# KVM-Explorer/AscendPathTracing

Hardware: AMD Instinct MI355X
Metric: Mray/s (ray segments per second) at 1920x1080, 8 bounces, 256 spp, demo scene (higher is better)
Workload: dtype f32; 1 GPU; C2: gen_spheres() 8-sphere scene, 1920x1080, S=64 (256 spp), depth 8, rays generated on device (counter RNG, seed 0), K-mode arithmetic, all segments traced (no retirement); segments_per_gpu=4246732800, parallelism=single GPU

## Files before the change

ascendpathtracing_amd/csrc/apt_host.h:

```cpp
#pragma once
#include <stdint.h>

#include <mutex>

#include "../../include/render_mi355x.h"

#define APT_API __attribute__((visibility("default")))

namespace apt {

void clear_error();
int set_error(int code, const char *fmt, const char *detail = "");

constexpr uint32_t kDefaultRefillLanes = 32;
constexpr int kMaxStatusDevices = 16;

struct Debug {
    uint32_t queue_ppw = 0;
    uint32_t queue_nbuf = 0;
    uint32_t queue_lds_pad = 0;
    uint32_t grid_walk = 0;
    double grid_spheres_per_cell = 0;
};

}

struct apt_context {
    struct Values {
        apt_render_params params;
        unsigned long long *trace_counter;
        uint32_t refill_lanes;
        apt::Debug debug;
        bool has_camera = false;
        apt_camera camera;
    };
    apt_context();
    Values snapshot();
    void set_params(const apt_render_params &p);
    void set_trace_counter(unsigned long long *c);
    void set_refill_lanes(uint32_t lanes);
    void set_camera(const apt_camera *cam_or_null);
    int set_debug(const char *key, double value);
    int get_debug(const char *key, double *value);
// ... 15 lines not shown
```

ascendpathtracing_amd/csrc/host_helpers.cpp:

```cpp
#include <stdint.h>
#include <stdio.h>
#include <string.h>

#include <algorithm>
#include <cmath>
#include <cstdlib>
#include <vector>

#include <string>

#include "../../include/render_mi355x.h"
#include "apt_host.h"
#include "pt_core.h"
#include "pt_camera.h"
#include "pt_leaf.h"

namespace {
thread_local std::string t_err;
thread_local int t_status = APT_OK;
}

namespace apt {
void clear_error() { t_err.clear(); t_status = APT_OK; }
int set_error(int code, const char *fmt, const char *detail) {
// ... 3 lines not shown
    t_status = code;
    return code;
}
apt_context &default_context() {
    static apt_context ctx;
    return ctx;
}
}

namespace {
double env_number(const char *name) {
    const char *e = getenv(name);
    return e ? atof(e) : 0.0;
}
}

apt_context::apt_context() {
    apt_default_params(&v_.params);
    v_.trace_counter = nullptr;
    v_.refill_lanes = apt::kDefaultRefillLanes;
    v_.has_camera = false;
    memset(&v_.camera, 0, sizeof v_.camera);
    struct { const char *env, *key; } knobs[] = {{"APT_QUEUE_PPW", "queue_ppw"}, {"APT_QUEUE_NBUF", "queue_nbuf"}, {"APT_QUEUE_LDS_PAD", "queue_lds_pad"},
                                                 {"APT_GRID_SPHERES_PER_CELL", "grid_spheres_per_cell"}};
    for (const auto &k : knobs) {
        const double v = env_number(k.env);
        if (v != 0.0) (void)set_debug(k.key, v);
    }
    if (const char *e = getenv("APT_GRID_WALK")) if (e[0] == 'i') v_.debug.grid_walk = 1;
    apt::clear_error();
}
apt_context::Values apt_context::snapshot() { std::lock_guard<std::mutex> g(m_); return v_; }
void apt_context::set_params(const apt_render_params &p) { std::lock_guard<std::mutex> g(m_); v_.params = p; }
void apt_context::set_trace_counter(unsigned long long *c) { std::lock_guard<std::mutex> g(m_); v_.trace_counter = c; }
void apt_context::set_refill_lanes(uint32_t lanes) { std::lock_guard<std::mutex> g(m_); v_.refill_lanes = lanes; }
void apt_context::set_camera(const apt_camera *cam) {
    std::lock_guard<std::mutex> g(m_);
    v_.has_camera = cam != nullptr;
    if (cam) v_.camera = *cam;
}
int apt_context::set_debug(const char *key, double value) {
    if (!key) return apt::set_error(APT_ERR_ARG, "apt_context_set_debug: key is null%s");
    const std::string k(key);
    const bool whole = value == std::floor(value);
    std::lock_guard<std::mutex> g(m_);
    apt::Debug &d = v_.debug;
    if (k == "queue_ppw") { if (!(whole && value >= 0 && value <= 4096)) goto range; d.queue_ppw = (uint32_t)value; }
    else if (k == "queue_nbuf") { if (!(whole && (value == 0 || (value >= 2 && value <= 16)))) goto range; d.queue_nbuf = (uint32_t)value; }
    else if (k == "queue_lds_pad") { if (!(whole && value >= 0 && value <= 32768)) goto range; d.queue_lds_pad = (uint32_t)value; }
    else if (k == "grid_walk") { if (!(value == 0 || value == 1)) goto range; d.grid_walk = (uint32_t)value; }
    else if (k == "grid_spheres_per_cell") { if (!(value == 0 || (value > 0.01 && value < 1e6))) goto range; d.grid_spheres_per_cell = value; }
    else return apt::set_error(APT_ERR_ARG, "apt_context_set_debug: unknown key '%s'", key);
    return APT_OK;
range:
    return apt::set_error(APT_ERR_ARG, "apt_context_set_debug: value out of range for '%s'", key);
}
int apt_context::get_debug(const char *key, double *value) {
    if (!key) return apt::set_error(APT_ERR_ARG, "apt_context_get_debug: key is null%s");
    const std::string k(key);
    std::lock_guard<std::mutex> g(m_);
    const apt::Debug &d = v_.debug;
    if (k == "queue_ppw") *value = d.queue_ppw;
    else if (k == "queue_nbuf") *value = d.queue_nbuf;
    else if (k == "queue_lds_pad") *value = d.queue_lds_pad;
    else if (k == "grid_walk") *value = d.grid_walk;
    else if (k == "grid_spheres_per_cell") *value = d.grid_spheres_per_cell;
    else return apt::set_error(APT_ERR_ARG, "apt_context_get_debug: unknown key '%s'", key);
    return APT_OK;
}
uint32_t *apt_context::status_lookup(int dev) {
    if (dev < 0 || dev >= apt::kMaxStatusDevices) return nullptr;
    std::lock_guard<std::mutex> g(m_);
    return status_[dev];
}
uint32_t *apt_context::status_adopt(int dev, uint32_t *fresh, uint32_t **spare) {
    *spare = nullptr;
    if (dev < 0 || dev >= apt::kMaxStatusDevices) { *spare = fresh; return nullptr; }
    std::lock_guard<std::mutex> g(m_);
    if (status_[dev]) *spare = fresh;
    else status_[dev] = fresh;
    return status_[dev];
}
void apt_context::status_release(uint32_t *out[apt::kMaxStatusDevices]) {
    std::lock_guard<std::mutex> g(m_);
    for (int i = 0; i < apt::kMaxStatusDevices; ++i) { out[i] = status_[i]; status_[i] = nullptr; }
}

// ... 531 lines not shown
```

ascendpathtracing_amd/csrc/materials.hip:

```cpp
#include <hip/hip_runtime.h>
#include <stdint.h>
#include <string.h>

#include <algorithm>

#include "../../include/render_mi355x.h"
#include "apt_materials.h"
#include "pt_core.h"
#include "pt_dispatch.h"
#include "pt_materials.h"

namespace {

TraceArgs mat_trace_args(const apt::MatTrace &t) {
    TraceArgs ta;
    ta.ns = t.ns; ta.depth = t.depth; ta.light = t.light;
    ta.eps = t.eps; ta.gain = 0.0f; ta.traced = t.traced;
    ta.status = t.status;
    ta.refill_lanes = (uint32_t)(uintptr_t)t.lights;
    ta.grid = t.grid;
    ta.grid_walk = 0;
    ta.emission = (uint32_t)((uint64_t)(uintptr_t)t.lights >> 32);
    ta.rr_start = t.rr_start;
    ta.seed = t.seed;
// ... 35 lines not shown
    }
    if (acc) atomicAdd(res, acc);
    if (rej) atomicAdd(res + 1, rej);
    if (bad) atomicAdd(res + 2, bad);
    if (ray_rej) atomicAdd(res + 3, ray_rej);
    if (max_cert) atomicMax(res + 4, max_cert);
}

}

namespace apt {

void selftest_direction(void *stream, const double *d3, uint64_t count, uint64_t *result5, uint8_t *flags) {
    const uint64_t blocks = std::min<uint64_t>((count + kBlock - 1) / kBlock, 256 * 16);
    hipLaunchKernelGGL(selftest_direction_kernel, dim3((unsigned)blocks), dim3(kBlock), 0, (hipStream_t)stream, d3, count,
                       (unsigned long long *)result5, flags);
}

void mat_render_frame(const MatFrameCall &c) {
    FrameArgs fa;
    CameraEx cx;
    if (c.camera) { cx = camera_ex(*c.camera, c.width, c.height); fa.cam = cx.base; }
    else camera_init(fa.cam, c.width, c.height);
    fa.width = c.width; fa.height = c.height; fa.samples = c.samples; fa.seed = c.t.seed;
    fa.pixel_begin = c.pixel_begin; fa.pixel_count = c.pixel_count; fa.fb = c.fb; fa.fb_u8 = c.fb_u8;
    const TraceArgs ta = mat_trace_args(c.t);
    LeafProg lp;
    (void)make_leaf_plan(c.samples, lp);
    if (c.camera) memcpy(&lp.leaf[kCamTailLeaf], &cx.t, sizeof cx.t);
    const int group = c.samples >= 8 ? 8 : 1;
    const uint64_t blocks = (c.pixel_count * 4u * (uint64_t)group + kBlock - 1) / kBlock;
    const size_t lds = lp.nleaves > 1 ? (size_t)kMaxStack * 3 * kStackSlots * sizeof(float) : 0;
    hipStream_t st = (hipStream_t)c.stream;
    with_flag(c.t.ns == 8, [&](auto ns8) { with_flag(c.t.grid != nullptr, [&](auto gr) { with_flag(group == 8, [&](auto g8) {
        with_flag(c.t.nee, [&](auto nee) { with_flag(c.t.lights != nullptr, [&](auto lt) { with_flag(c.camera != nullptr, [&](auto cam) {
            hipLaunchKernelGGL((render_frame_mat_kernel<mat_scene_form(ns8, gr, nee, lt, cam), g8 ? 8 : 1>), dim3((unsigned)blocks), dim3(kBlock), lds,
                               st, c.spheres, c.materials, fa, ta, lp);
        }); }); });
    }); }); });
}

void mat_render_paths(const MatPathsCall &c) {
    const TraceArgs ta = mat_trace_args(c.t);
    const uint64_t blocks = (c.c + kBlock - 1) / kBlock;
    hipStream_t st = (hipStream_t)c.stream;
    with_flag(c.t.ns == 8, [&](auto ns8) { with_flag(c.t.grid != nullptr, [&](auto gr) {
        with_flag(c.t.nee, [&](auto nee) { with_flag(c.t.lights != nullptr, [&](auto lt) {
// ... 20 lines not shown
```

ascendpathtracing_amd/csrc/pt_core.h:

```cpp
#pragma once
#include <stdint.h>
#include <cmath>
#include <cstdlib>
#include <cstring>
#include <math.h>

#if defined(__HIPCC__)
#include <hip/hip_runtime.h>
#define APT_HD __host__ __device__ __forceinline__
#else
#define APT_HD inline
#endif

namespace apt {

constexpr int kModeKernel = 0;
constexpr int kModeOracle = 1;
constexpr float kMissT = 1e20f;

APT_HD float intersect_sphere(float cx, float cy, float cz, float r2, float ox, float oy, float oz, float dx, float dy,
                              float dz, float eps) {
    float ocx = cx - ox, ocy = cy - oy, ocz = cz - oz;
    float b = ocx * dx;
    b = b + ocy * dy;
// ... 371 lines not shown
    uint32_t b;
    memcpy(&b, &f, sizeof b);
    return b;
#endif
}
APT_HD uint32_t dir_probe(double d0, double d1, double d2, double y, float e0, float e1, float e2, double &cert) {
    double q0, q1, q2, Z;
    uint32_t mid;
    fast_direction(d0, d1, d2, norm3_sq(d0, d1, d2), y, q0, q1, q2, Z, cert, mid);
    const bool ray = (fabs(d0) >= 0x1p-60) & (fabs(d1) >= 0x1p-60) & (fabs(d2) >= 0x1p-60) & (Z >= 0x1p-60) & (fabs(cert) <= kDirCertTau);
    uint32_t r = ray ? 64u : 0u;
    r |= (ray & (dir_mid_key(q0) > 16u * kDirMidD)) ? 1u : 0u;
    r |= (ray & (dir_mid_key(q1) > 16u * kDirMidD)) ? 2u : 0u;
    r |= (ray & (dir_mid_key(q2) > 16u * kDirMidD)) ? 4u : 0u;
    r |= float_bits((float)q0) != float_bits(e0) ? 8u : 0u;
    r |= float_bits((float)q1) != float_bits(e1) ? 16u : 0u;
    r |= float_bits((float)q2) != float_bits(e2) ? 32u : 0u;
    return r;
}
struct RayCheck { double lo, cert; uint32_t mid; };
APT_HD bool ray_check_ok(const RayCheck &k) { return (k.lo >= 0x1p-60) & (fabs(k.cert) <= kDirCertTau) & (k.mid > 16u * kDirMidD); }
APT_HD bool ray_check_ok_rn(const RayCheck &k) { return (k.lo >= 0x1p-60) & (k.cert <= 0x1p60); }

template <bool FAST, bool RSQDIR = true, class CAM>
APT_HD void camera_ray_t(const CAM &c, uint32_t w, uint32_t h, uint32_t i, uint32_t j, uint32_t sy, uint32_t sx,
                         double u1, double u2, float &rox, float &roy, float &roz, float &rdx, float &rdy, float &rdz, RayCheck &chk) {
    double arg1, arg2;
    const double ddx = tent_t<FAST>(u1, arg1), ddy = tent_t<FAST>(u2, arg2);
    const double xa = ((double)sx + 0.5 + ddx) / 2 + (double)i, xb = ((double)sy + 0.5 + ddy) / 2 + (double)j;
    double a, b;
#if defined(__HIP_DEVICE_COMPILE__)
    if (FAST) {
        a = div_by_rn_reciprocal(xa, (double)w, c.inv_w) - 0.5;
        b = div_by_rn_reciprocal(xb, (double)h, c.inv_h) - 0.5;
    } else
#endif
    {
        a = xa / (double)w - 0.5;
        b = xb / (double)h - 0.5;
    }
    const double d0 = cam_cx0(c) * a;
    const double d1 = cam_cy1(c) * b + cam_g1(c);
    const double d2 = cam_cy2(c) * b + cam_g2(c);
    const double n2 = norm3_sq(d0, d1, d2);
    rox = (float)(c.pos[0] + d0 * 140);
    roy = (float)(c.pos[1] + d1 * 140);
    roz = (float)(c.pos[2] + d2 * 140);
#if defined(__HIP_DEVICE_COMPILE__)
// ... 8 lines not shown
        lo = min3_abs_f64(lo, d1, d2);
        asm("v_min_f64 %0, %1, %2" : "=v"(lo) : "v"(lo), "v"(n2));
        chk.lo = lo; chk.cert = n;
        return;
    }
    if (FAST) {
        double q0, q1, q2, Z;
        fast_direction(d0, d1, d2, n2, __builtin_amdgcn_rsq(n2), q0, q1, q2, Z, chk.cert, chk.mid);
        rdx = (float)q0; rdy = (float)q1; rdz = (float)q2;
        double lo = min3_abs_f64(arg1, arg2, xa);
        lo = min3_abs_f64(lo, xb, d0);
        lo = min3_abs_f64(lo, d1, d2);
        asm("v_min_f64 %0, %1, %2" : "=v"(lo) : "v"(lo), "v"(Z));
        chk.lo = lo;
        return;
    }
#endif
    const double n = sqrt(n2);
    rdx = (float)(d0 / n);
    rdy = (float)(d1 / n);
    rdz = (float)(d2 / n);
}

template <bool RSQDIR = true, class CAM>
APT_HD void camera_ray(const CAM &c, uint32_t w, uint32_t h, uint32_t i, uint32_t j, uint32_t sy, uint32_t sx,
                       double u1, double u2, float &rox, float &roy, float &roz, float &rdx, float &rdy, float &rdz) {
    RayCheck chk;
#if defined(__HIP_DEVICE_COMPILE__)
    camera_ray_t<true, RSQDIR>(c, w, h, i, j, sy, sx, u1, u2, rox, roy, roz, rdx, rdy, rdz, chk);
    if (__builtin_expect(__builtin_amdgcn_ballot_w64(!(RSQDIR ? ray_check_ok(chk) : ray_check_ok_rn(chk))) == 0, 1)) return;
    asm volatile("" ::: "memory");
#endif
    camera_ray_t<false>(c, w, h, i, j, sy, sx, u1, u2, rox, roy, roz, rdx, rdy, rdz, chk);
}
APT_HD Ray camera_ray(const Camera &c, uint32_t w, uint32_t h, uint32_t i, uint32_t j, uint32_t sy, uint32_t sx,
                      double u1, double u2) {
    Ray r;
    camera_ray(c, w, h, i, j, sy, sx, u1, u2, r.ox, r.oy, r.oz, r.dx, r.dy, r.dz);
    return r;
}

APT_HD uint64_t splitmix64(uint64_t x) {
    x += 0x9E3779B97F4A7C15ull;
    x = (x ^ (x >> 30)) * 0xBF58476D1CE4E5B9ull;
    x = (x ^ (x >> 27)) * 0x94D049BB133111EBull;
    return x ^ (x >> 31);
}
APT_HD uint64_t xorshift64s(uint64_t &s) {
// ... 12 lines not shown
    return d - 1.0;
#endif
}
constexpr uint64_t kPathStride = 0x3C6EF372FE94F82Aull;
APT_HD void path_uniforms_at(uint64_t state, double &u1, double &u2) {
    u1 = unit_from_bits(splitmix64(state));
    u2 = unit_from_bits(splitmix64(state + 0x9E3779B97F4A7C15ull));
}
APT_HD void path_uniforms(uint64_t seed, uint64_t path, double &u1, double &u2) {
    path_uniforms_at(splitmix64(seed) + path * kPathStride, u1, u2);
}

constexpr uint64_t kPairStateStep = 8ull * kPathStride;
APT_HD uint64_t lane_base_state(uint64_t seed, uint64_t pbase, uint32_t j) { return splitmix64(seed) + (pbase + j) * kPathStride; }
APT_HD uint64_t chain_state_uniform(uint64_t lane_base, uint32_t u) {
    uint64_t off = (uint64_t)u * kPathStride;
#if defined(__HIP_DEVICE_COMPILE__)
    asm("" : "+s"(off));
#endif
    return lane_base + off;
}

#if defined(__HIPCC__)
template <class CAM>
__device__ __forceinline__ void camera_ray_pair(const CAM &c, uint32_t w, uint32_t h, uint32_t i, uint32_t j, uint32_t sy, uint32_t sx,
                                                uint64_t state_a, f2 &ox, f2 &oy, f2 &oz, f2 &dx, f2 &dy, f2 &dz) {
#if defined(__HIP_DEVICE_COMPILE__)
    double u1a, u2a, u1b, u2b;
    path_uniforms_at(state_a, u1a, u2a);
    path_uniforms_at(state_a + kPairStateStep, u1b, u2b);
    float ax, ay, az, adx, ady, adz, bx, by, bz, bdx, bdy, bdz;
    RayCheck ka, kb;
    camera_ray_t<true>(c, w, h, i, j, sy, sx, u1a, u2a, ax, ay, az, adx, ady, adz, ka);
    camera_ray_t<true>(c, w, h, i, j, sy, sx, u1b, u2b, bx, by, bz, bdx, bdy, bdz, kb);
    double lo;
    asm("v_min_f64 %0, %1, %2" : "=v"(lo) : "v"(ka.lo), "v"(kb.lo));
    const bool ok = (lo >= 0x1p-60) & (fabs(ka.cert) <= kDirCertTau) & (fabs(kb.cert) <= kDirCertTau) &
                    ((ka.mid < kb.mid ? ka.mid : kb.mid) > 16u * kDirMidD);
    if (__builtin_expect(__builtin_amdgcn_ballot_w64(!ok) != 0, 0)) {
        asm volatile("" ::: "memory");
        camera_ray_t<false>(c, w, h, i, j, sy, sx, u1a, u2a, ax, ay, az, adx, ady, adz, ka);
        camera_ray_t<false>(c, w, h, i, j, sy, sx, u1b, u2b, bx, by, bz, bdx, bdy, bdz, kb);
    }
    ox = f2{ax, bx}; oy = f2{ay, by}; oz = f2{az, bz};
    dx = f2{adx, bdx}; dy = f2{ady, bdy}; dz = f2{adz, bdz};
#endif
}
#endif
// ... 172 lines not shown
```

ascendpathtracing_amd/csrc/pt_frame.h:

```cpp
#pragma once
#include "pt_trace.h"

namespace {

struct FrameArgs {
    Camera cam;
    uint32_t width, height, samples;
    uint64_t seed;
    uint64_t pixel_begin, pixel_count;
    float *fb;
    uint8_t *fb_u8;
};

__device__ __forceinline__ void park_camera(Camera &cam, const FrameArgs &fa) {
    if (threadIdx.x < sizeof(Camera) / sizeof(double)) (&cam.pos[0])[threadIdx.x] = (&fa.cam.pos[0])[threadIdx.x];
}

template <int GROUP>
struct FrameLane {
    uint32_t j, sub;
    uint64_t pl;
    bool valid;
    uint64_t q;
    uint32_t pi, pj, sy, sx;
    uint64_t pbase;
};
template <int GROUP>
__device__ __forceinline__ FrameLane<GROUP> frame_lane(const FrameArgs &fa, uint32_t tid = threadIdx.x) {
    FrameLane<GROUP> f;
    const uint64_t L = (uint64_t)xcd_chunked_block<16>(blockIdx.x, gridDim.x) * kBlock + tid;
    f.j = (GROUP == 8) ? (uint32_t)(L & 7) : 0u;
    f.sub = (uint32_t)(L / GROUP) & 3u;
    f.pl = L / (4 * GROUP);
    f.valid = f.pl < fa.pixel_count;
    f.q = fa.pixel_begin + (f.valid ? f.pl : 0);
    f.pi = (uint32_t)(f.q / fa.height); f.pj = (uint32_t)(f.q % fa.height);
    f.sy = f.sub >> 1; f.sx = f.sub & 1;
    f.pbase = (f.q * 4 + f.sub) * fa.samples;
    return f;
}

constexpr uint32_t frame_u8_words(int group) { return kBlock / (4 * group) * 3 / 4; }
template <int GROUP>
__device__ __forceinline__ void frame_decode(const FrameArgs fa, uint64_t pl, bool valid, const float (&res)[3],
                                             uint32_t (&u8pack_kernel)[frame_u8_words(GROUP)]) {
    constexpr uint32_t kPixPerBlock = kBlock / (4 * GROUP), kU8Words = frame_u8_words(GROUP);
    typedef __attribute__((address_space(3))) uint8_t lds_uint8;
    typedef __attribute__((address_space(3))) uint32_t lds_uint32;
    lds_uint32 *const u8pack = (lds_uint32 *)u8pack_kernel;
    static_assert(kPixPerBlock * 3 % 4 == 0, "a workgroup's 8-bit pixels are whole dwords");
    const uint32_t lane = threadIdx.x & 63;
    const uint64_t pl0 = pl - (threadIdx.x / (4 * GROUP));
    const bool pack = fa.fb_u8 && pl0 + kPixPerBlock <= fa.pixel_count && (((uintptr_t)fa.fb_u8 + pl0 * 3) & 3u) == 0;
    const float fs = (float)fa.samples;
    const int gbase = (int)(lane & ~(uint32_t)(4 * GROUP - 1));
#pragma unroll
    for (int ch = 0; ch < 3; ++ch) {
        const float mean = res[ch] / fs;
        double acc = 0.0;
#pragma unroll
        for (int sq = 0; sq < 4; ++sq) acc = acc + (double)__shfl(mean, gbase + sq * GROUP, 64);
        const double v = acc / 4;
        const double cl = v < 0 ? 0 : (v > 1 ? 1 : v);
        if (valid && (lane & (4 * GROUP - 1)) == 0) {
            fa.fb[(uint64_t)ch * fa.pixel_count + pl] = (float)cl;
            const uint8_t b8 = (uint8_t)(cl * 255);
            if (pack) ((lds_uint8 *)u8pack)[(threadIdx.x / (4 * GROUP)) * 3 + ch] = b8;
            else if (fa.fb_u8) fa.fb_u8[pl * 3 + ch] = b8;
        }
    }
    if (pack) {
        __syncthreads();
        if (threadIdx.x < kU8Words) reinterpret_cast<uint32_t *>(fa.fb_u8 + pl0 * 3)[threadIdx.x] = u8pack[threadIdx.x];
    }
}

}
```

ascendpathtracing_amd/csrc/pt_kernels.h:

```cpp
#pragma once
#include "pt_trace.h"
#include "pt_trace2.h"
#include "pt_queue.h"
#include "pt_frame_mt.h"

namespace {

template <int MODE, int SC, bool RETIRE>
__global__ __launch_bounds__(kBlock, SC == kSceneGrid ? APT_GRID_WAVES : 1) void render_paths_kernel(const float *__restrict__ rays,
                                                              const float *__restrict__ sph,
                                                              float *__restrict__ colors, uint64_t n_total,
                                                              uint64_t begin, uint64_t count, TraceArgs ta) {
    constexpr bool NS8 = SC == kScene8;
    static_assert(!(RETIRE && NS8), "APT_FLAG_RETIRE on the 8-sphere scene is render_paths_queue_kernel's");
    __shared__ float4 tab[kTab8Floats4];
    __shared__ float4 tile[SC == kSceneTiles ? kTile : 1];
    Scene8 sc;
    Tab8 tab8{tab, tab + 8};
    if (NS8) tab8 = load_scene8(sph, sc, tab);
    const uint64_t local = (uint64_t)blockIdx.x * kBlock + threadIdx.x;
    const bool valid = local < count;
    const uint64_t p = begin + (valid ? local : 0);
    PathState s;
    path_init(s, rays[p], rays[n_total + p], rays[2 * n_total + p], rays[3 * n_total + p], rays[4 * n_total + p],
// ... 144 lines not shown
}

template <int MODE, int SC, int GROUP, bool RETIRE, bool TWO = false>
__global__ __launch_bounds__(kBlock, TWO ? APT_TWO_WAVES : (SC == kSceneGrid ? APT_GRID_WAVES : (SC == kSceneTiles ? APT_TILE_WAVES : APT_FULL_WAVES))) void render_frame_kernel(const float *__restrict__ sph, FrameArgs fa,
                                                              TraceArgs ta, LeafProg lp) {
    constexpr bool NS8 = SC == kScene8;
    static_assert(!(RETIRE && NS8 && GROUP == 8), "APT_FLAG_RETIRE on the 8-sphere scene with samples >= 8 is render_frame_queue8_kernel's (pt_queue.h)");
    if (SC == kSceneGrid && ta.grid_walk == 2u && grid_queue_usable(ta)) return;
    __shared__ float4 tab[kTab8Floats4];
    __shared__ float4 tile[SC == kSceneTiles ? kTile : 1];
    extern __shared__ float dyn_lds[];
    float *stack_lds = dyn_lds;
    float *queue_lds = dyn_lds + (lp.nleaves > 1 ? kMaxStack * 3 * kStackSlots : 0);
    __shared__ Camera cam;
    park_camera(cam, fa);
    Scene8 sc;
    Tab8 tab8{tab, tab + 8};
    if (NS8) tab8 = load_scene8(sph, sc, tab);
    else __syncthreads();
    const bool planes = NS8 && sc.planes;
    (void)planes;

    const uint32_t lane = threadIdx.x & 63;
    const FrameLane<GROUP> fl = frame_lane<GROUP>(fa);
    const uint32_t j = fl.j, sub = fl.sub;
    const uint64_t pl = fl.pl;
    const bool valid = fl.valid;
    const uint32_t pi = fl.pi, pj = fl.pj, sy = fl.sy, sx = fl.sx;
    const uint64_t pbase = fl.pbase;
    uint32_t traced = 0;
    uint32_t queue_traced = 0;

    const Gain3 gain = load_gain(sph, ta);
    struct Col { float r, g, b; };
    auto sample = [&](uint32_t k) __attribute__((always_inline)) -> Col {
        uint64_t pb = pbase;
        if (TWO) {
            uint32_t tid = threadIdx.x;
            asm volatile("" : "+v"(tid));
            pb = frame_lane<GROUP>(fa, tid).pbase;
        }
        double u1, u2;
        path_uniforms(fa.seed, pb + k, u1, u2);
        float rox, roy, roz, rdx, rdy, rdz;
        camera_ray(cam, fa.width, fa.height, pi, pj, sy, sx, u1, u2, rox, roy, roz, rdx, rdy, rdz);
        PathState s;
        path_init(s, rox, roy, roz, rdx, rdy, rdz);
        if (SC == kScene8) traced += trace_ns8<MODE, RETIRE>(sc, tab8, s, valid, ta, pb + k);
        else if (SC == kSceneGrid) traced += trace_grid<MODE, RETIRE>(sph, ta.grid, s, valid, ta, pb + k);
        else traced += trace_dyn<MODE, RETIRE>(sph, tile, s, valid, ta, pb + k);
        return Col{s.rxy.x * gain.r, s.rxy.y * gain.g, s.rz * gain.b};
    };
    auto add = [](const Col &a, const Col &b) { return Col{a.r + b.r, a.g + b.g, a.b + b.b}; };
    struct Col2 { Col a, b; };
    const uint64_t lane_state = TWO ? lane_base_state(fa.seed, pbase, j) : 0;
    auto sample2 = [&](uint32_t u) __attribute__((always_inline)) -> Col2 {
        PathPair pp;
        camera_ray_pair(cam, fa.width, fa.height, pi, pj, sy, sx, chain_state_uniform(lane_state, u), pp.ox, pp.oy, pp.oz, pp.dx, pp.dy, pp.dz);
        asm("" : "+v"(pp.ox), "+v"(pp.oy), "+v"(pp.oz), "+v"(pp.dx), "+v"(pp.dy), "+v"(pp.dz));
        pp.rx = pp.ry = pp.rz = f2{1.0f, 1.0f};
        trace2_ns8<MODE>(sc, tab8, pp, ta, planes);
        traced += 2 * ta.depth;
        return Col2{Col{pp.rx.x * gain.r, pp.ry.x * gain.g, pp.rz.x * gain.b}, Col{pp.rx.y * gain.r, pp.ry.y * gain.g, pp.rz.y * gain.b}};
    };

    float res[3] = {0.0f, 0.0f, 0.0f};
    uint32_t start = 0;
    int sp = 0;
    for (uint32_t leaf = 0; leaf < lp.nleaves; ++leaf) {
        const uint32_t n = lp.len(leaf);
        float acc[3];
        if (GROUP == 1) {
            Col a = {0.0f, 0.0f, 0.0f};
            for (uint32_t k = 0; k < n; ++k) a = add(a, sample(start + k));
            acc[0] = a.r; acc[1] = a.g; acc[2] = a.b;
        } else {
            const uint32_t nfull = n & ~7u;
            if (RETIRE && SC == kSceneTiles) {
                float *colq = queue_lds + (size_t)(threadIdx.x >> 6) * 3u * 8u * lp.maxleaf;
                const uint32_t total = 8u * nfull;
                const uint32_t qstride = 8u * lp.maxleaf;
                uint32_t next = 0;
                uint32_t depth_left = 0, cur_item = 0, slot_item = 0;
                uint64_t cur_key = 0, slot_key = 0;
                uint32_t n_bounce_exec = 0, n_gen_exec = 0;
                float sl_ox = 0.f, sl_oy = 0.f, sl_oz = 0.f, sl_dx = 0.f, sl_dy = 0.f, sl_dz = 1.f;
                bool slot_full = false, slot_valid = false, cur_valid = false;
                PathState s;
                path_init(s, 0.f, 0.f, 0.f, 0.f, 0.f, 1.f);
                auto refill = [&](PathState &cur) -> bool {
                    for (;;) {
                        const bool want = !slot_full;
                        const unsigned long long wants = __ballot(want);
                        const bool busy_any = __any(depth_left != 0 || slot_full);
                        if (next < total && wants && ((uint32_t)__popcll(wants) >= ta.refill_lanes || !busy_any)) {
                            ++n_gen_exec;
                            const uint32_t rank = __builtin_amdgcn_mbcnt_hi((uint32_t)(wants >> 32),
                                                  __builtin_amdgcn_mbcnt_lo((uint32_t)wants, 0u));
                            const uint32_t remaining = total - next;
                            const bool take = want && rank < remaining;
                            const uint32_t item = take ? next + rank : 0u;
                            const uint32_t g = item / nfull, k = item - g * nfull;
                            const int src = (int)(8u * g);
                            const uint32_t gpi = __shfl(pi, src, 64), gpj = __shfl(pj, src, 64);
                            const uint32_t gsub = __shfl(sub, src, 64);
                            const uint32_t blo = __shfl((uint32_t)pbase, src, 64), bhi = __shfl((uint32_t)(pbase >> 32), src, 64);
                            const bool gvalid = __shfl((int)valid, src, 64) != 0;
                            if (take) {
                                slot_valid = gvalid;
                                double u1, u2;
                                const uint64_t path = (((uint64_t)bhi << 32) | blo) + start + k;
                                if (ta.rr_start) slot_key = rr_path_key(ta.seed, path);
                                path_uniforms(fa.seed, path, u1, u2);
                                camera_ray(cam, fa.width, fa.height, gpi, gpj, gsub >> 1, gsub & 1u, u1, u2, sl_ox, sl_oy, sl_oz, sl_dx,
                                           sl_dy, sl_dz);
                                slot_item = item;
                                slot_full = true;
                            }
                            next += min((uint32_t)__popcll(wants), remaining);
                        }
                        const bool begin = depth_left == 0 && slot_full;
                        if (begin) {
                            cur.oxy = f2{sl_ox, sl_oy}; cur.oz = sl_oz; cur.dxy = f2{sl_dx, sl_dy}; cur.dz = sl_dz;
                            cur.rxy = f2{1.0f, 1.0f}; cur.rz = 1.0f; cur.alive = 1u;
                            cur_item = slot_item;
                            cur_key = slot_key;
                            cur_valid = slot_valid;
// ... 82 lines not shown
        start += n;
        if (lp.nleaves == 1) {
            res[0] = acc[0]; res[1] = acc[1]; res[2] = acc[2];
        } else {
#pragma unroll
            for (int ch = 0; ch < 3; ++ch) stack_lds[(sp * 3 + ch) * kStackSlots + (threadIdx.x >> 3)] = acc[ch];
            ++sp;
            for (uint32_t m = 0; m < lp.ncomb(leaf); ++m) {
                --sp;
#pragma unroll
                for (int ch = 0; ch < 3; ++ch) {
                    const float a = stack_lds[((sp - 1) * 3 + ch) * kStackSlots + (threadIdx.x >> 3)];
                    const float b = stack_lds[(sp * 3 + ch) * kStackSlots + (threadIdx.x >> 3)];
                    stack_lds[((sp - 1) * 3 + ch) * kStackSlots + (threadIdx.x >> 3)] = a + b;
                }
            }
        }
    }
    if (lp.nleaves > 1) {
#pragma unroll
        for (int ch = 0; ch < 3; ++ch) res[ch] = stack_lds[ch * kStackSlots + (threadIdx.x >> 3)];
    }

    __shared__ uint32_t u8pack[frame_u8_words(GROUP)];
    frame_decode<GROUP>(fa, pl, valid, res, u8pack);
    count_traced(ta, (valid ? traced : 0) + queue_traced);
}

__global__ __launch_bounds__(kBlock) void test_scene_kernel(const float *__restrict__ rays,
                                                            const float *__restrict__ sph, float *__restrict__ out,
                                                            uint64_t n_total, uint32_t ns, int32_t light, float eps) {
    const uint64_t p = (uint64_t)blockIdx.x * kBlock + threadIdx.x;
    if (p >= n_total) return;
    const float ox = rays[p], oy = rays[n_total + p], oz = rays[2 * n_total + p];
    const float dx = rays[3 * n_total + p], dy = rays[4 * n_total + p], dz = rays[5 * n_total + p];
    float mind = kMissT;
    int id = -1;
    for (uint32_t k = 0; k < ns; ++k)
        test_scene_sphere(sph[ns + k], sph[2 * (size_t)ns + k], sph[3 * (size_t)ns + k], sph[k], ox, oy, oz, dx, dy, dz,
                          eps, (int)k, mind, id);
#pragma unroll
    for (int c = 0; c < 3; ++c) {
        float v = 0.0f;
        if (id >= 0) v = (id == light) ? sph[(size_t)(4 + c) * ns + id] : sph[(size_t)(7 + c) * ns + id];
        out[(uint64_t)c * n_total + p] = v;
    }
}

__global__ __launch_bounds__(kBlock) void gen_rays_kernel(Camera cam, uint32_t width, uint32_t height,
// ... 349 lines not shown
```

ascendpathtracing_amd/csrc/render_kernels.hip:

```cpp
#include <hip/hip_runtime.h>
#include <algorithm>
#include <new>
#include <stdint.h>
#include <stdio.h>
#include <stdlib.h>
#include <string.h>
#include <string>
#include <type_traits>
#include <vector>

#include "../../include/render_mi355x.h"
#include "apt_host.h"
#include "apt_materials.h"
#include "pt_core.h"
#include "pt_dispatch.h"

#include "pt_kernels.h"
#include "pt_grid_build.h"

namespace {

using apt::clear_error;
int fail(int code, const char *fmt, const char *detail = "") { return apt::set_error(code, fmt, detail); }
int hip_fail(hipError_t e) { return fail(APT_ERR_DEVICE, "HIP: %s", hipGetErrorString(e)); }
// ... 88 lines not shown
    const uint32_t *lights = m.with_lights ? static_cast<const uint32_t *>(m.lights) : nullptr;
    return apt::MatTrace{ta.ns, ta.depth, ta.rr_start, ta.light, !lights && (p->flags & APT_FLAG_NEE) != 0, ta.eps, ta.seed, ta.status ? ta.grid : nullptr, ta.status, ta.traced, lights};
}

struct PathRange {
    uint64_t n_image, b, c;
    bool band;
    uint64_t plane() const { return band ? c : n_image; }
    template <class T> T *base(T *buf) const { return band ? buf - b : buf; }
};
int path_range(const apt_render_params *p, PathRange &r) {
    r.n_image = (uint64_t)p->width * p->height * 4u * p->samples;
    r.b = p->path_begin;
    if (r.b > r.n_image) return fail(APT_ERR_ARG, "path_begin beyond the image%s");
    r.c = p->path_count ? p->path_count : r.n_image - r.b;
    if (r.b + r.c > r.n_image) return fail(APT_ERR_ARG, "path range beyond the image%s");
    r.band = p->flags & APT_FLAG_BAND_BUFFERS;
    return APT_OK;
}

FrameArgs make_frame_args(const apt_render_params *p, uint64_t pixel_begin, uint64_t pixel_count, float *fb, uint8_t *fb_u8) {
    FrameArgs fa;
    camera_init(fa.cam, p->width, p->height);
    fa.width = p->width; fa.height = p->height; fa.samples = p->samples; fa.seed = p->seed;
    fa.pixel_begin = pixel_begin; fa.pixel_count = pixel_count; fa.fb = fb; fa.fb_u8 = fb_u8;
    return fa;
}

size_t sphere_table_bytes(uint32_t num_spheres) { return ((size_t)num_spheres * 10 + 127) / 128 * 128 * sizeof(float); }

constexpr uint64_t kTwoPathBufferMin = 1ull << 20;

int do_render_paths(const Launch &ls, const apt_render_params *p, void *stream, const float *rays,
                    const float *spheres, float *colors, bool mat = false, const MatArgs &ma = MatArgs()) {
    int rc = check_params(p, mat);
    if (rc) return rc;
    if (mat && (rc = check_mat_args(p, ma))) return rc;
    if (!rays || !spheres || !colors) return fail(APT_ERR_ARG, "rays/spheres/colors must be non-null%s");
    PathRange r;
    if ((rc = path_range(p, r)) || r.c == 0) return rc;
    const uint64_t n = r.plane(), b = r.b, c = r.c;
    const uint64_t blocks = (c + kBlock - 1) / kBlock;
    if (blocks > 0x7fffffffull) return fail(APT_ERR_ARG, "path_count too large for one launch; shard it%s");
    if (mat) {
        if ((rc = check_lights_status(ma, ls.status))) return rc;
        apt::mat_render_paths(apt::MatPathsCall{make_mat_trace(p, ls, ma), r.base(rays), spheres, ma.materials, r.base(colors), n, b, c, stream});
        return launched();
// ... 18 lines not shown
            hipLaunchKernelGGL((render_paths_kernel<m, kScene8, false>), grid, dim3(kBlock), 0, st, rays, spheres, colors, n, b, c, ta);
        } else {
            with_flag(ta.grid != nullptr, [&](auto gr) { with_flag(retire, [&](auto rt) {
                hipLaunchKernelGGL((render_paths_kernel<m, gr ? kSceneGrid : kSceneTiles, rt>), grid, dim3(kBlock), 0, st, rays, spheres, colors, n, b, c, ta);
            }); });
        }
    });
    return launched();
}

bool queue_launch_shape(const apt::Debug &dbg, const LeafProg &lp, bool rr, bool grid, uint64_t pixel_count, bool retire, QueueArgs &qa,
                        uint64_t &waves, size_t &qlds) {
    const uint32_t subs = queue_unit_subs(grid), unit_items = subs * lp.maxleaf, window = subs == 4u ? 512u : 384u;
    qa.nbuf = dbg.queue_nbuf ? dbg.queue_nbuf : std::max(2u, std::min(16u, (window + unit_items - 1u) / unit_items));
    qa.buf_bytes = queue_buf_bytes(lp.maxleaf, subs);
    qa.retire = retire ? 1u : 0u;
    const uint64_t ppw = dbg.queue_ppw ? dbg.queue_ppw : std::max<uint64_t>(4, std::min<uint64_t>(16, pixel_count / 8192u));
    qa.ppw = (uint32_t)ppw;
    waves = (pixel_count + ppw - 1) / ppw;
    qlds = queue_lds_bytes(queue_pool_entries(grid), rr, qa.nbuf, lp.nleaves > 1, qa.buf_bytes, subs) + dbg.queue_lds_pad;
    return waves <= 0x7fffffffull;
}

int do_render_frame(const Launch &ls, const apt_render_params *p, void *stream, const float *spheres,
                    uint64_t pixel_begin, uint64_t pixel_count, float *fb, uint8_t *fb_u8, bool mat = false,
                    const MatArgs &ma = MatArgs()) {
    int rc = check_params(p, mat);
    if (rc) return rc;
    if (mat && (rc = check_mat_args(p, ma))) return rc;
    if (!spheres || !fb) return fail(APT_ERR_ARG, "spheres/fb must be non-null%s");
    const uint64_t npix = (uint64_t)p->width * p->height;
    if (pixel_begin > npix || pixel_count > npix - pixel_begin) return fail(APT_ERR_ARG, "pixel range beyond the image%s");
    if (pixel_count == 0) return APT_OK;
    LeafProg lp;
    if ((rc = make_leaf_prog(p->samples, lp))) return rc;
    const int group = p->samples >= 8 ? 8 : 1;
    const uint64_t lanes = pixel_count * 4u * (uint64_t)group;
    const uint64_t blocks = (lanes + kBlock - 1) / kBlock;
    if (blocks > 0x7fffffffull) return fail(APT_ERR_ARG, "pixel_count too large for one launch; shard it%s");
    const apt::Debug &dbg = ls.cv.debug;
    if (mat) {
        if ((rc = check_lights_status(ma, ls.status))) return rc;
        if (ls.cv.has_camera && !apt::mat_camera_fits(p->samples)) return fail(APT_ERR_ARG, "camera: a frame with a camera set takes a pairwise-sum plan of at most 44 leaves (every samples <= 4199 has one)%s");
        apt::mat_render_frame(apt::MatFrameCall{make_mat_trace(p, ls, ma), spheres, ma.materials, p->width, p->height, p->samples, pixel_begin,
                                                pixel_count, fb, fb_u8, stream, ls.cv.has_camera ? &ls.cv.camera : nullptr});
        return launched();
    }
    if ((rc = refuse_camera(ls.cv, "render_frame"))) return rc;
    hipStream_t st = (hipStream_t)stream;
    const bool ns8 = p->num_spheres == 8;
    TraceArgs ta = make_trace_args(p, ls);
    const FrameArgs fa = make_frame_args(p, pixel_begin, pixel_count, fb, fb_u8);
    const bool retire = p->flags & APT_FLAG_RETIRE, rrk = ta.rr_start != 0;
    if (retire && ns8 && group == 8 && p->depth > 0) {
        QueueArgs qa;
        uint64_t waves;
        size_t qlds;
        if (!queue_launch_shape(dbg, lp, rrk, false, pixel_count, true, qa, waves, qlds)) return fail(APT_ERR_ARG, "pixel_count too large for one launch; shard it%s");
        with_mode(p->mode, [&](auto m) { with_flag(rrk, [&](auto rr) {
            hipLaunchKernelGGL((render_frame_queue8_kernel<m, rr>), dim3((unsigned)waves), dim3(64), qlds, st, spheres, fa, ta, lp, qa);
        }); });
        return launched();
    }
    if (!ns8 && ta.grid && group == 8 && p->depth > 0 && dbg.grid_walk != 1u) {
        QueueArgs qa;
        uint64_t waves;
        size_t qlds;
        if (!queue_launch_shape(dbg, lp, rrk, true, pixel_count, retire, qa, waves, qlds)) return fail(APT_ERR_ARG, "pixel_count too large for one launch; shard it%s");
        const bool vouched = (p->flags & APT_FLAG_GRID_SLOTS) && eps_allows_rootkey(p->eps) && ta.status != nullptr;
        TraceArgs ta_q = ta;
        ta_q.grid_walk = vouched ? 3u : 0u;
        with_mode(p->mode, [&](auto m) { with_flag(rrk, [&](auto rr) { with_flag(ta.traced != nullptr, [&](auto stats) {
            hipLaunchKernelGGL((render_frame_queue8_kernel<m, rr, kSceneGrid, stats>), dim3((unsigned)waves), dim3(64), qlds, st, spheres, fa, ta_q, lp, qa);
        }); }); });
        if ((rc = launched()) || vouched) return rc;
        ta.grid_walk = 2;
    }
    size_t lds = lp.nleaves > 1 ? (size_t)kMaxStack * 3 * kStackSlots * sizeof(float) : 0;
    if (retire && !ns8 && !ta.grid && group == 8) lds += (size_t)(kBlock / 64) * 3 * 8 * lp.maxleaf * sizeof(float);
    const dim3 grid((unsigned)blocks);
    with_mode(p->mode, [&](auto m) {
        if (ns8 && group == 8) {
            if (!retire && !rrk && p->samples >= 16)
                hipLaunchKernelGGL((render_frame_kernel<m, kScene8, 8, false, true>), grid, dim3(kBlock), lds, st, spheres, fa, ta, lp);
            else
                hipLaunchKernelGGL((render_frame_kernel<m, kScene8, 8, false>), grid, dim3(kBlock), lds, st, spheres, fa, ta, lp);
        } else if (ns8) {
            with_flag(retire, [&](auto rt) {
                hipLaunchKernelGGL((render_frame_kernel<m, kScene8, 1, rt>), grid, dim3(kBlock), lds, st, spheres, fa, ta, lp);
            });
        } else {
            with_flag(ta.grid != nullptr, [&](auto gr) { with_flag(group == 8, [&](auto g8) { with_flag(retire, [&](auto rt) {
                hipLaunchKernelGGL((render_frame_kernel<m, gr ? kSceneGrid : kSceneTiles, g8 ? 8 : 1, rt>), grid, dim3(kBlock), lds, st, spheres, fa, ta, lp);
            }); }); });
        }
    });
    return launched();
}

void split_range(uint64_t total, uint64_t r, uint64_t parts, uint64_t &begin, uint64_t &count) {
    const uint64_t base = total / parts, extra = total % parts;
    begin = r * base + (r < extra ? r : extra);
    count = base + (r < extra ? 1 : 0);
// ... 616 lines not shown
```

Measured before the change: 222,700 Mray/s.

## Process multiple pixel blocks per workgroup in rounds with LDS-parked results

Each workgroup now loops over up to eight consecutive pixel blocks (rounds), parking per-pixel sums in LDS and decoding/writing all of them to the framebuffer at the end. The grid shrinks accordingly, and pixel coordinates, path bases and RNG lane state advance incrementally per round. Frame args are reloaded from the kernarg segment to limit register pressure. This is meant to amortise block launch, setup and framebuffer-write overhead, at the cost of extra LDS and possibly worse tail balance with fewer blocks.

```diff
diff --git a/ascendpathtracing_amd/csrc/apt_host.h b/ascendpathtracing_amd/csrc/apt_host.h
--- a/ascendpathtracing_amd/csrc/apt_host.h
+++ b/ascendpathtracing_amd/csrc/apt_host.h
@@ -19,6 +19,7 @@
     uint32_t queue_ppw = 0;
     uint32_t queue_nbuf = 0;
     uint32_t queue_lds_pad = 0;
+    uint32_t frame_rounds = 0;
     uint32_t grid_walk = 0;
     double grid_spheres_per_cell = 0;
 };
diff --git a/ascendpathtracing_amd/csrc/host_helpers.cpp b/ascendpathtracing_amd/csrc/host_helpers.cpp
--- a/ascendpathtracing_amd/csrc/host_helpers.cpp
+++ b/ascendpathtracing_amd/csrc/host_helpers.cpp
@@ -49,7 +49,7 @@
     v_.has_camera = false;
     memset(&v_.camera, 0, sizeof v_.camera);
     struct { const char *env, *key; } knobs[] = {{"APT_QUEUE_PPW", "queue_ppw"}, {"APT_QUEUE_NBUF", "queue_nbuf"}, {"APT_QUEUE_LDS_PAD", "queue_lds_pad"},
-                                                 {"APT_GRID_SPHERES_PER_CELL", "grid_spheres_per_cell"}};
+                                                 {"APT_GRID_SPHERES_PER_CELL", "grid_spheres_per_cell"}, {"APT_FRAME_ROUNDS", "frame_rounds"}};
     for (const auto &k : knobs) {
         const double v = env_number(k.env);
         if (v != 0.0) (void)set_debug(k.key, v);
@@ -75,6 +75,7 @@
     if (k == "queue_ppw") { if (!(whole && value >= 0 && value <= 4096)) goto range; d.queue_ppw = (uint32_t)value; }
     else if (k == "queue_nbuf") { if (!(whole && (value == 0 || (value >= 2 && value <= 16)))) goto range; d.queue_nbuf = (uint32_t)value; }
     else if (k == "queue_lds_pad") { if (!(whole && value >= 0 && value <= 32768)) goto range; d.queue_lds_pad = (uint32_t)value; }
+    else if (k == "frame_rounds") { if (!(whole && value >= 0 && value <= 16)) goto range; d.frame_rounds = (uint32_t)value; }
     else if (k == "grid_walk") { if (!(value == 0 || value == 1)) goto range; d.grid_walk = (uint32_t)value; }
     else if (k == "grid_spheres_per_cell") { if (!(value == 0 || (value > 0.01 && value < 1e6))) goto range; d.grid_spheres_per_cell = value; }
     else return apt::set_error(APT_ERR_ARG, "apt_context_set_debug: unknown key '%s'", key);
@@ -90,6 +91,7 @@
     if (k == "queue_ppw") *value = d.queue_ppw;
     else if (k == "queue_nbuf") *value = d.queue_nbuf;
     else if (k == "queue_lds_pad") *value = d.queue_lds_pad;
+    else if (k == "frame_rounds") *value = d.frame_rounds;
     else if (k == "grid_walk") *value = d.grid_walk;
     else if (k == "grid_spheres_per_cell") *value = d.grid_spheres_per_cell;
     else return apt::set_error(APT_ERR_ARG, "apt_context_get_debug: unknown key '%s'", key);
diff --git a/ascendpathtracing_amd/csrc/materials.hip b/ascendpathtracing_amd/csrc/materials.hip
--- a/ascendpathtracing_amd/csrc/materials.hip
+++ b/ascendpathtracing_amd/csrc/materials.hip
@@ -81,7 +81,7 @@
     CameraEx cx;
     if (c.camera) { cx = camera_ex(*c.camera, c.width, c.height); fa.cam = cx.base; }
     else camera_init(fa.cam, c.width, c.height);
-    fa.width = c.width; fa.height = c.height; fa.samples = c.samples; fa.seed = c.t.seed;
+    fa.width = c.width; fa.height = c.height; fa.samples = c.samples; fa.rounds = 1; fa.seed = c.t.seed;
     fa.pixel_begin = c.pixel_begin; fa.pixel_count = c.pixel_count; fa.fb = c.fb; fa.fb_u8 = c.fb_u8;
     const TraceArgs ta = mat_trace_args(c.t);
     LeafProg lp;
diff --git a/ascendpathtracing_amd/csrc/pt_core.h b/ascendpathtracing_amd/csrc/pt_core.h
--- a/ascendpathtracing_amd/csrc/pt_core.h
+++ b/ascendpathtracing_amd/csrc/pt_core.h
@@ -417,8 +417,8 @@
 APT_HD bool ray_check_ok(const RayCheck &k) { return (k.lo >= 0x1p-60) & (fabs(k.cert) <= kDirCertTau) & (k.mid > 16u * kDirMidD); }
 APT_HD bool ray_check_ok_rn(const RayCheck &k) { return (k.lo >= 0x1p-60) & (k.cert <= 0x1p60); }
 
-template <bool FAST, bool RSQDIR = true, class CAM>
-APT_HD void camera_ray_t(const CAM &c, uint32_t w, uint32_t h, uint32_t i, uint32_t j, uint32_t sy, uint32_t sx,
+template <bool FAST, bool RSQDIR = true, class CAM, class IJ>
+APT_HD void camera_ray_t(const CAM &c, uint32_t w, uint32_t h, IJ i, IJ j, uint32_t sy, uint32_t sx,
                          double u1, double u2, float &rox, float &roy, float &roz, float &rdx, float &rdy, float &rdz, RayCheck &chk) {
     double arg1, arg2;
     const double ddx = tent_t<FAST>(u1, arg1), ddy = tent_t<FAST>(u2, arg2);
@@ -473,8 +473,8 @@
     rdz = (float)(d2 / n);
 }
 
-template <bool RSQDIR = true, class CAM>
-APT_HD void camera_ray(const CAM &c, uint32_t w, uint32_t h, uint32_t i, uint32_t j, uint32_t sy, uint32_t sx,
+template <bool RSQDIR = true, class CAM, class IJ>
+APT_HD void camera_ray(const CAM &c, uint32_t w, uint32_t h, IJ i, IJ j, uint32_t sy, uint32_t sx,
                        double u1, double u2, float &rox, float &roy, float &roz, float &rdx, float &rdy, float &rdz) {
     RayCheck chk;
 #if defined(__HIP_DEVICE_COMPILE__)
@@ -533,8 +533,8 @@
 }
 
 #if defined(__HIPCC__)
-template <class CAM>
-__device__ __forceinline__ void camera_ray_pair(const CAM &c, uint32_t w, uint32_t h, uint32_t i, uint32_t j, uint32_t sy, uint32_t sx,
+template <class CAM, class IJ>
+__device__ __forceinline__ void camera_ray_pair(const CAM &c, uint32_t w, uint32_t h, IJ i, IJ j, uint32_t sy, uint32_t sx,
                                                 uint64_t state_a, f2 &ox, f2 &oy, f2 &oz, f2 &dx, f2 &dy, f2 &dz) {
 #if defined(__HIP_DEVICE_COMPILE__)
     double u1a, u2a, u1b, u2b;
diff --git a/ascendpathtracing_amd/csrc/pt_frame.h b/ascendpathtracing_amd/csrc/pt_frame.h
--- a/ascendpathtracing_amd/csrc/pt_frame.h
+++ b/ascendpathtracing_amd/csrc/pt_frame.h
@@ -6,6 +6,7 @@
 struct FrameArgs {
     Camera cam;
     uint32_t width, height, samples;
+    uint32_t rounds;
     uint64_t seed;
     uint64_t pixel_begin, pixel_count;
     float *fb;
@@ -26,9 +27,10 @@
     uint64_t pbase;
 };
 template <int GROUP>
-__device__ __forceinline__ FrameLane<GROUP> frame_lane(const FrameArgs &fa, uint32_t tid = threadIdx.x) {
+__device__ __forceinline__ FrameLane<GROUP> frame_lane(const FrameArgs &fa, uint32_t tid = threadIdx.x,
+                                                        uint32_t blk = xcd_chunked_block<16>(blockIdx.x, gridDim.x)) {
     FrameLane<GROUP> f;
-    const uint64_t L = (uint64_t)xcd_chunked_block<16>(blockIdx.x, gridDim.x) * kBlock + tid;
+    const uint64_t L = (uint64_t)blk * kBlock + tid;
     f.j = (GROUP == 8) ? (uint32_t)(L & 7) : 0u;
     f.sub = (uint32_t)(L / GROUP) & 3u;
     f.pl = L / (4 * GROUP);
@@ -75,4 +77,85 @@
     }
 }
 
+constexpr bool frame_kernel_takes_rounds(int group, bool retire) { return !(group == 1 && retire); }
+constexpr uint32_t frame_park_floats(int group, uint32_t rounds) { return rounds * (kBlock / group) * 3; }
+constexpr uint32_t frame_rounds_lds_bytes(int group, uint32_t rounds) {
+    return frame_park_floats(group, rounds) * 4 + rounds * (kBlock / (4 * group)) * 3;
 }
+typedef const __attribute__((address_space(4))) FrameArgs *FrameArgsReload;
+__device__ __forceinline__ FrameArgsReload frame_args_reload() {
+    const __attribute__((address_space(4))) char *k = (const __attribute__((address_space(4))) char *)__builtin_amdgcn_kernarg_segment_ptr();
+    asm volatile("" : "+s"(k));
+    return (FrameArgsReload)(k + sizeof(const float *));
+}
+static_assert(alignof(FrameArgs) == sizeof(const float *), "FrameArgs follows the kernel's first argument without padding");
+constexpr uint32_t kFrameItemPixels = 21;
+
+template <int GROUP>
+__device__ __forceinline__ void frame_park(float *park_generic, uint32_t round, uint32_t tid, const float (&res)[3]) {
+    typedef __attribute__((address_space(3))) float lds_float;
+    lds_float *const park = (lds_float *)park_generic;
+    if (tid % GROUP == 0) {
+#pragma unroll
+        for (int ch = 0; ch < 3; ++ch) park[(round * (kBlock / GROUP) + tid / GROUP) * 3 + ch] = res[ch];
+    }
+}
+
+template <int GROUP>
+__device__ __forceinline__ void frame_decode_rounds(FrameArgsReload kfa, uint32_t blk0, bool takes_rounds, float *park_generic) {
+    const uint32_t rounds = takes_rounds ? kfa->rounds : 1u, samples = kfa->samples;
+    const uint64_t pixel_count = kfa->pixel_count;
+    float *const fb = kfa->fb;
+    uint8_t *const fb_u8 = kfa->fb_u8;
+    constexpr uint32_t P = kBlock / (4 * GROUP), PW = 64 / (4 * GROUP), kSlots = kBlock / GROUP;
+    typedef __attribute__((address_space(3))) float lds_float;
+    typedef __attribute__((address_space(3))) uint8_t lds_uint8;
+    typedef __attribute__((address_space(3))) uint32_t lds_uint32;
+    lds_float *const park = (lds_float *)park_generic;
+    lds_uint32 *const u8pack = (lds_uint32 *)(park + frame_park_floats(GROUP, rounds));
+    __builtin_amdgcn_fence(__ATOMIC_RELEASE, "wavefront");
+    __builtin_amdgcn_wave_barrier();
+    __builtin_amdgcn_fence(__ATOMIC_ACQUIRE, "wavefront");
+    const uint32_t lane = threadIdx.x & 63, wave = threadIdx.x >> 6;
+    const uint64_t pl0 = (uint64_t)blk0 * P;
+    const uint32_t wg_pixels = P * rounds;
+    const bool pack = fb_u8 && pl0 + wg_pixels <= pixel_count && (((uintptr_t)fb_u8 + pl0 * 3) & 3u) == 0;
+    const float fs = (float)samples;
+    const bool pow2 = (samples & (samples - 1u)) == 0u;
+    const float rfs = 1.0f / fs;
+    const uint32_t wave_pixels = PW * rounds;
+    for (uint32_t first = 0; first < wave_pixels; first += kFrameItemPixels) {
+        const uint32_t c = min(wave_pixels - first, kFrameItemPixels);
+        const uint32_t ch = (lane >= c ? 1u : 0u) + (lane >= 2u * c ? 1u : 0u);
+        const uint32_t pw = first + lane - ch * c;
+        const uint32_t r = pw / PW, k = pw % PW;
+        const uint32_t off = r * P + wave * PW + k;
+        const uint64_t pl = pl0 + off;
+        if (lane < 3u * c && pl < pixel_count) {
+            const lds_float *const sums = park + (r * kSlots + wave * (64 / GROUP) + k * 4) * 3 + ch;
+            float mean[4];
+            if (pow2) {
+#pragma unroll
+                for (int sq = 0; sq < 4; ++sq) mean[sq] = sums[sq * 3] * rfs;
+            } else {
+#pragma unroll
+                for (int sq = 0; sq < 4; ++sq) mean[sq] = sums[sq * 3] / fs;
+            }
+            double acc = 0.0;
+#pragma unroll
+            for (int sq = 0; sq < 4; ++sq) acc = acc + (double)mean[sq];
+            const double v = acc / 4;
+            const double cl = v < 0 ? 0 : (v > 1 ? 1 : v);
+            fb[(uint64_t)ch * pixel_count + pl] = (float)cl;
+            const uint8_t b8 = (uint8_t)(cl * 255);
+            if (pack) ((lds_uint8 *)u8pack)[off * 3 + ch] = b8;
+            else if (fb_u8) fb_u8[pl * 3 + ch] = b8;
+        }
+    }
+    if (pack) {
+        __syncthreads();
+        for (uint32_t t = threadIdx.x; t < wg_pixels * 3 / 4; t += kBlock) reinterpret_cast<uint32_t *>(fb_u8 + pl0 * 3)[t] = u8pack[t];
+    }
+}
+
+}
diff --git a/ascendpathtracing_amd/csrc/pt_kernels.h b/ascendpathtracing_amd/csrc/pt_kernels.h
--- a/ascendpathtracing_amd/csrc/pt_kernels.h
+++ b/ascendpathtracing_amd/csrc/pt_kernels.h
@@ -190,12 +190,16 @@
     (void)planes;
 
     const uint32_t lane = threadIdx.x & 63;
-    const FrameLane<GROUP> fl = frame_lane<GROUP>(fa);
+    constexpr uint32_t kPixPerBlock = kBlock / (4 * GROUP);
+    constexpr bool kRounds = frame_kernel_takes_rounds(GROUP, RETIRE);
+    const uint32_t blk0 = xcd_chunked_block<16>(blockIdx.x, gridDim.x) * (kRounds ? fa.rounds : 1u);
+    uint32_t blk = blk0;
+    const FrameLane<GROUP> fl = frame_lane<GROUP>(fa, threadIdx.x, blk0);
     const uint32_t j = fl.j, sub = fl.sub;
-    const uint64_t pl = fl.pl;
-    const bool valid = fl.valid;
-    const uint32_t pi = fl.pi, pj = fl.pj, sy = fl.sy, sx = fl.sx;
-    const uint64_t pbase = fl.pbase;
+    bool valid = fl.valid;
+    double pid = (double)fl.pi, pjd = (double)fl.pj;
+    const uint32_t sy = fl.sy, sx = fl.sx;
+    uint64_t pbase = fl.pbase;
     uint32_t traced = 0;
     uint32_t queue_traced = 0;
 
@@ -206,12 +210,12 @@
         if (TWO) {
             uint32_t tid = threadIdx.x;
             asm volatile("" : "+v"(tid));
-            pb = frame_lane<GROUP>(fa, tid).pbase;
+            pb = frame_lane<GROUP>(fa, tid, blk).pbase;
         }
         double u1, u2;
         path_uniforms(fa.seed, pb + k, u1, u2);
         float rox, roy, roz, rdx, rdy, rdz;
-        camera_ray(cam, fa.width, fa.height, pi, pj, sy, sx, u1, u2, rox, roy, roz, rdx, rdy, rdz);
+        camera_ray(cam, fa.width, fa.height, pid, pjd, sy, sx, u1, u2, rox, roy, roz, rdx, rdy, rdz);
         PathState s;
         path_init(s, rox, roy, roz, rdx, rdy, rdz);
         if (SC == kScene8) traced += trace_ns8<MODE, RETIRE>(sc, tab8, s, valid, ta, pb + k);
@@ -221,10 +225,10 @@
     };
     auto add = [](const Col &a, const Col &b) { return Col{a.r + b.r, a.g + b.g, a.b + b.b}; };
     struct Col2 { Col a, b; };
-    const uint64_t lane_state = TWO ? lane_base_state(fa.seed, pbase, j) : 0;
+    uint64_t lane_state = TWO ? lane_base_state(fa.seed, pbase, j) : 0;
     auto sample2 = [&](uint32_t u) __attribute__((always_inline)) -> Col2 {
         PathPair pp;
-        camera_ray_pair(cam, fa.width, fa.height, pi, pj, sy, sx, chain_state_uniform(lane_state, u), pp.ox, pp.oy, pp.oz, pp.dx, pp.dy, pp.dz);
+        camera_ray_pair(cam, fa.width, fa.height, pid, pjd, sy, sx, chain_state_uniform(lane_state, u), pp.ox, pp.oy, pp.oz, pp.dx, pp.dy, pp.dz);
         asm("" : "+v"(pp.ox), "+v"(pp.oy), "+v"(pp.oz), "+v"(pp.dx), "+v"(pp.dy), "+v"(pp.dz));
         pp.rx = pp.ry = pp.rz = f2{1.0f, 1.0f};
         trace2_ns8<MODE>(sc, tab8, pp, ta, planes);
@@ -232,6 +236,9 @@
         return Col2{Col{pp.rx.x * gain.r, pp.ry.x * gain.g, pp.rz.x * gain.b}, Col{pp.rx.y * gain.r, pp.ry.y * gain.g, pp.rz.y * gain.b}};
     };
 
+    float *const park_lds = queue_lds + (RETIRE && SC == kSceneTiles && GROUP == 8 ? (kBlock / 64) * 3u * 8u * lp.maxleaf : 0u);
+    uint32_t round = 0;
+    for (;;) {
     float res[3] = {0.0f, 0.0f, 0.0f};
     uint32_t start = 0;
     int sp = 0;
@@ -270,7 +277,7 @@
                             const uint32_t item = take ? next + rank : 0u;
                             const uint32_t g = item / nfull, k = item - g * nfull;
                             const int src = (int)(8u * g);
-                            const uint32_t gpi = __shfl(pi, src, 64), gpj = __shfl(pj, src, 64);
+                            const uint32_t gpi = __shfl((uint32_t)pid, src, 64), gpj = __shfl((uint32_t)pjd, src, 64);
                             const uint32_t gsub = __shfl(sub, src, 64);
                             const uint32_t blo = __shfl((uint32_t)pbase, src, 64), bhi = __shfl((uint32_t)(pbase >> 32), src, 64);
                             const bool gvalid = __shfl((int)valid, src, 64) != 0;
@@ -399,9 +406,32 @@
         for (int ch = 0; ch < 3; ++ch) res[ch] = stack_lds[ch * kStackSlots + (threadIdx.x >> 3)];
     }
 
-    __shared__ uint32_t u8pack[frame_u8_words(GROUP)];
-    frame_decode<GROUP>(fa, pl, valid, res, u8pack);
-    count_traced(ta, (valid ? traced : 0) + queue_traced);
+    uint32_t tid = threadIdx.x;
+    asm volatile("" : "+v"(tid));
+    frame_park<GROUP>(park_lds, round, tid, res);
+    if (ta.traced) {
+        const uint32_t t = (valid ? traced : 0) + queue_traced;
+        if (t) atomicAdd(ta.traced, (unsigned long long)t);
+    }
+    traced = 0; queue_traced = 0;
+    ++round;
+    blk = (uint32_t)__builtin_amdgcn_readfirstlane((int)(blk + 1u));
+    const FrameArgsReload kfa = frame_args_reload();
+    const uint64_t pixel_count = kfa->pixel_count;
+    if (!kRounds || round >= kfa->rounds || (uint64_t)blk * kPixPerBlock >= pixel_count) break;
+    const uint32_t height = kfa->height;
+    uint32_t col_step = 0, row_step = kPixPerBlock;
+    while (row_step >= height) { row_step -= height; ++col_step; }
+    const uint64_t path_step = 4ull * kPixPerBlock * kfa->samples;
+    valid = (uint64_t)blk * kPixPerBlock + tid / (4 * GROUP) < pixel_count;
+    if (valid) {
+        pid += (double)col_step; pjd += (double)row_step;
+        if (pjd >= (double)height) { pjd -= (double)height; pid += 1.0; }
+        pbase += path_step;
+        lane_state += path_step * kPathStride;
+    }
+    }
+    frame_decode_rounds<GROUP>(frame_args_reload(), blk - round, kRounds, park_lds);
 }
 
 __global__ __launch_bounds__(kBlock) void test_scene_kernel(const float *__restrict__ rays,
diff --git a/ascendpathtracing_amd/csrc/render_kernels.hip b/ascendpathtracing_amd/csrc/render_kernels.hip
--- a/ascendpathtracing_amd/csrc/render_kernels.hip
+++ b/ascendpathtracing_amd/csrc/render_kernels.hip
@@ -134,7 +134,7 @@
 FrameArgs make_frame_args(const apt_render_params *p, uint64_t pixel_begin, uint64_t pixel_count, float *fb, uint8_t *fb_u8) {
     FrameArgs fa;
     camera_init(fa.cam, p->width, p->height);
-    fa.width = p->width; fa.height = p->height; fa.samples = p->samples; fa.seed = p->seed;
+    fa.width = p->width; fa.height = p->height; fa.samples = p->samples; fa.rounds = 1; fa.seed = p->seed;
     fa.pixel_begin = pixel_begin; fa.pixel_count = pixel_count; fa.fb = fb; fa.fb_u8 = fb_u8;
     return fa;
 }
@@ -199,6 +199,15 @@
     return waves <= 0x7fffffffull;
 }
 
+constexpr uint32_t kFrameRoundsMax = 8, kFrameRoundsRefills = 16;
+uint32_t frame_rounds(const apt::Debug &dbg, int group, bool retire, uint64_t blocks) {
+    if (!frame_kernel_takes_rounds(group, retire)) return 1u;
+    if (dbg.frame_rounds) return group == 8 ? dbg.frame_rounds : std::min(dbg.frame_rounds, 8u);
+    uint32_t r = group == 8 ? kFrameRoundsMax : 1u;
+    while (r > 1u && blocks / r < kFrameRoundsRefills * 1024ull) r /= 2u;
+    return r;
+}
+
 int do_render_frame(const Launch &ls, const apt_render_params *p, void *stream, const float *spheres,
                     uint64_t pixel_begin, uint64_t pixel_count, float *fb, uint8_t *fb_u8, bool mat = false,
                     const MatArgs &ma = MatArgs()) {
@@ -227,7 +236,7 @@
     hipStream_t st = (hipStream_t)stream;
     const bool ns8 = p->num_spheres == 8;
     TraceArgs ta = make_trace_args(p, ls);
-    const FrameArgs fa = make_frame_args(p, pixel_begin, pixel_count, fb, fb_u8);
+    FrameArgs fa = make_frame_args(p, pixel_begin, pixel_count, fb, fb_u8);
     const bool retire = p->flags & APT_FLAG_RETIRE, rrk = ta.rr_start != 0;
     if (retire && ns8 && group == 8 && p->depth > 0) {
         QueueArgs qa;
@@ -255,7 +264,9 @@
     }
     size_t lds = lp.nleaves > 1 ? (size_t)kMaxStack * 3 * kStackSlots * sizeof(float) : 0;
     if (retire && !ns8 && !ta.grid && group == 8) lds += (size_t)(kBlock / 64) * 3 * 8 * lp.maxleaf * sizeof(float);
-    const dim3 grid((unsigned)blocks);
+    fa.rounds = frame_rounds(dbg, group, retire, blocks);
+    lds += frame_rounds_lds_bytes(group, fa.rounds);
+    const dim3 grid((unsigned)((blocks + fa.rounds - 1) / fa.rounds));
     with_mode(p->mode, [&](auto m) {
         if (ns8 && group == 8) {
             if (!retire && !rrk && p->samples >= 16)
```

Result: no change. 222,500 Mray/s, median of 2 (-0.1%).
